# liamliaw/medical-image-segmentation-with-visual-prompts

Measured on AMD Instinct MI355X. Metric: 3D volumes/sec (96^3, bf16) training step, higher is better.
Workload: dtype bf16; 1 GPU; cfg1: swin_unetr downstream, 1-ch 96^3, batch 4/GPU, window (7, 7, 7), enc_prompt=False, dec_prompt=False, dropout 0.0, random-init weights; global_batch=4, parallelism=dp1, launch=eager (one C-ABI call per kernel)

## Files before the change

### medical-image-segmentation-with-visual-prompts_amd/csrc/swin_fwd.hip

```cpp
#include "swin_common.hpp"

template <int KS, bool CH12>
__global__ __launch_bounds__(256, 4) void k_swin_qkv_fwd(MivpSwinDesc d, const bf16_t* __restrict__ x,
                                                      const int* __restrict__ tok_src,
                                                      const float* __restrict__ ln_w, const float* __restrict__ ln_b,
                                                      const bf16_t* __restrict__ wqkv,
                                                      bf16_t* __restrict__ q, bf16_t* __restrict__ k,
                                                      bf16_t* __restrict__ v) {
    const int lane = threadIdx.x & 63, wave = __builtin_amdgcn_readfirstlane(threadIdx.x >> 6);
    const int r = lane & 15, g = lane >> 4;
    const int C = d.C, hd = C / d.heads;
    const long T = (long)d.B * d.P * d.Nqp;
    const long tile0 = ((long)blockIdx.x * 4 + wave) * 2;

    bf16x8 xb[2][KS];
    long bp[2];
    int slot[2];
    bool live[2];
#pragma unroll
    for (int u = 0; u < 2; ++u) {
        const long t = (tile0 + u) * 16 + r;
        live[u] = t < T;
        const unsigned tt = live[u] ? (unsigned)t : 0u;
        const unsigned bpu = tt / (unsigned)d.Nqp;
        bp[u] = bpu;
        slot[u] = (int)(tt - bpu * (unsigned)d.Nqp);
        const int pw = (int)(bpu % (unsigned)d.P);
        const long b = bpu / (unsigned)d.P;
        const int src = live[u] ? tok_src[pw * d.Nqp + slot[u]] : -2;
        float xs[KS][8];
        float sum = 0.f;
#pragma unroll
        for (int s = 0; s < KS; ++s) {
            const int c = 32 * s + 8 * g;
            if (src >= 0 && c < C) {
                bf16x8 raw = ld8(x + ((b * d.vol_in + src) * (long)C + c));
#pragma unroll
                for (int i = 0; i < 8; ++i) { xs[s][i] = (float)raw[i]; sum += xs[s][i]; }
            } else {
#pragma unroll
                for (int i = 0; i < 8; ++i) xs[s][i] = 0.f;
            }
        }
        const float mean = col_sum(sum) / (float)C;
        float var = 0.f;
#pragma unroll
        for (int s = 0; s < KS; ++s) {
            if (32 * s + 8 * g < C) {
#pragma unroll
                for (int i = 0; i < 8; ++i) { const float dv = xs[s][i] - mean; var += dv * dv; }
            }
        }
        const float rstd = rsqrtf(col_sum(var) / (float)C + d.ln_eps);
#pragma unroll
        for (int s = 0; s < KS; ++s) {
            const int c = 32 * s + 8 * g;
            bf16x8 y = zero8();
            if (src >= -1 && c < C) {
#pragma unroll
                for (int i = 0; i < 8; ++i) y[i] = (bf16_t)((xs[s][i] - mean) * rstd * ln_w[c + i] + ln_b[c + i]);
            }
            xb[u][s] = y;
        }
    }

    if constexpr (CH12) {
        const unsigned Nqp = (unsigned)d.Nqp;
        if (tile0 * 16 >= T) return;
        long chunk[2];
#pragma unroll
        for (int u = 0; u < 2; ++u) {
            const unsigned tt = (unsigned)((tile0 + u) * 16);
            const unsigned bpu = (unsigned)__builtin_amdgcn_readfirstlane((int)(tt / Nqp));
            chunk[u] = ((long)bpu * 4 * Nqp + (tt - bpu * Nqp)) * 12;
        }
        const int dl = lane < 48 ? lane : lane - 16, rq = dl / 3, gq = dl - 3 * rq;
        int src_addr[4];
        bool from_b[4];
#pragma unroll
        for (int h = 0; h < 4; ++h) {
            const int ch = 12 * h + 4 * gq;
            src_addr[h] = 4 * (rq + 16 * ((ch & 15) >> 2));
            from_b[h] = (ch >> 4) != ((12 * h) >> 4);
        }
#pragma unroll
        for (int sl = 0; sl < 3; ++sl) {
            const float sc = sl == 0 ? d.q_scale : (sl == 1 ? MIVP_LOG2E : 1.0f);
            u32x2 pk[3][2];
#pragma unroll
            for (int t = 0; t < 3; ++t) {
                f32x4 acc0 = fzero4(), acc1 = fzero4();
#pragma unroll
                for (int s = 0; s < KS; ++s) {
                    const char* fb = reinterpret_cast<const char*>(wqkv) + (size_t)(((3 * sl + t) * KS + s) * 1024);
                    const bf16x8 a = *reinterpret_cast<const bf16x8*>(fb + (unsigned)(16 * lane));
                    acc0 = mfma16(a, xb[0][s], acc0);
                    acc1 = mfma16(a, xb[1][s], acc1);
                }
                pk[t][0] = __builtin_bit_cast(u32x2, pack4(acc0 * sc));
                pk[t][1] = __builtin_bit_cast(u32x2, pack4(acc1 * sc));
            }
            bf16_t* base = sl == 0 ? q : (sl == 1 ? k : v);
#pragma unroll
            for (int h = 0; h < 4; ++h) {
                const int ta = (12 * h) >> 4, tb = (12 * h + 8) >> 4;
#pragma unroll
                for (int u = 0; u < 2; ++u) {
                    u32x2 piece;
                    piece[0] = (unsigned)__builtin_amdgcn_ds_bpermute(src_addr[h], (int)pk[ta][u][0]);
                    piece[1] = (unsigned)__builtin_amdgcn_ds_bpermute(src_addr[h], (int)pk[ta][u][1]);
                    if (tb != ta) {
                        const unsigned b0 = (unsigned)__builtin_amdgcn_ds_bpermute(src_addr[h], (int)pk[tb][u][0]);
                        const unsigned b1 = (unsigned)__builtin_amdgcn_ds_bpermute(src_addr[h], (int)pk[tb][u][1]);
                        piece[0] = from_b[h] ? b0 : piece[0];
                        piece[1] = from_b[h] ? b1 : piece[1];
                    }
                    char* cb = reinterpret_cast<char*>(base + (chunk[u] + (long)h * Nqp * 12));
                    *reinterpret_cast<u32x2*>(cb + (unsigned)(8 * dl)) = piece;
                }
            }
        }
        return;
    }
    const int n_out = 3 * C;
    const int n_tiles = (n_out + 15) / 16;
    const int per_split = (n_tiles + gridDim.y - 1) / gridDim.y;
    const int nt_begin = blockIdx.y * per_split;
    const int nt_end = nt_begin + per_split < n_tiles ? nt_begin + per_split : n_tiles;
    constexpr bool LDSW = KS >= 3;
    constexpr int PCS = (64 * KS + 255) / 256;
    __shared__ __attribute__((aligned(16))) char wsm[LDSW ? 2 * KS * 1024 : 16];
    using WR = OperandRows<32>;
    bf16x8 wreg[PCS];
    auto slab_fetch = [&](int nt) {
#pragma unroll
        for (int u = 0; u < PCS; ++u) {
            wreg[u] = ld8(wqkv + (long)nt * KS * 512 + 8 * min((int)threadIdx.x + 256 * u, 64 * KS - 1));
        }
    };
    auto slab_store = [&](int buf) {
#pragma unroll
        for (int u = 0; u < PCS; ++u) {
            *reinterpret_cast<bf16x8*>(wsm + buf * KS * 1024 + 16 * min((int)threadIdx.x + 256 * u, 64 * KS - 1)) = wreg[u];
        }
    };
    if (LDSW && nt_begin < nt_end) { slab_fetch(nt_begin); slab_store(0); __syncthreads(); }
    int o_sel = (16 * nt_begin + 4 * g) / C;
    int o_head = ((16 * nt_begin + 4 * g) - o_sel * C) / hd;
    int o_j0 = (16 * nt_begin + 4 * g) - o_sel * C - o_head * hd;
    for (int nt = nt_begin; nt < nt_end; ++nt) {
        f32x4 acc0 = fzero4(), acc1 = fzero4();
        const int nrow = 16 * nt + r;
        if (LDSW) {
            const int cur = (nt - nt_begin) & 1;
            if (nt + 1 < nt_end) slab_fetch(nt + 1);
            const char* slab = wsm + cur * KS * 1024;
#pragma unroll
            for (int s = 0; s < KS; ++s) {
                const bf16x8 a = *reinterpret_cast<const bf16x8*>(slab + s * 1024 + 16 * lane);
                acc0 = mfma16(a, xb[0][s], acc0);
                acc1 = mfma16(a, xb[1][s], acc1);
            }
            if (nt + 1 < nt_end) slab_store(cur ^ 1);
            __syncthreads();
        } else {
#pragma unroll
            for (int s = 0; s < KS; ++s) {
                const bf16x8 a = wfrag(wqkv, KS, nt, s, lane);
                acc0 = mfma16(a, xb[0][s], acc0);
                acc1 = mfma16(a, xb[1][s], acc1);
            }
        }
        const int n0 = 16 * nt + 4 * g;
        if (n0 < n_out) {
            while (o_j0 >= hd) { o_j0 -= hd; ++o_head; }
            while (o_head >= d.heads) { o_head -= d.heads; ++o_sel; }
            const int sel = o_sel, head = o_head, j0 = o_j0;
            o_j0 += 16;
            bf16_t* base = sel == 0 ? q : (sel == 1 ? k : v);
            const float sc = sel == 0 ? d.q_scale : (sel == 1 ? MIVP_LOG2E : 1.0f);
            if (live[0]) st4(base + ((bp[0] * d.heads + head) * d.Nqp + slot[0]) * (long)hd + j0, pack4(acc0 * sc));
            if (live[1]) st4(base + ((bp[1] * d.heads + head) * d.Nqp + slot[1]) * (long)hd + j0, pack4(acc1 * sc));
        }
    }
}

__global__ __launch_bounds__(256) void k_prompt_kv_fwd(MivpSwinDesc d, const float* __restrict__ prompt,
                                                       const float* __restrict__ ln_w, const float* __restrict__ ln_b,
                                                       const bf16_t* __restrict__ wqkv, bf16_t* __restrict__ kp,
                                                       bf16_t* __restrict__ vp, float* __restrict__ yln) {
    extern __shared__ __attribute__((aligned(16))) char smem[];
    float* y = reinterpret_cast<float*>(smem);
    float* red = y + d.C;
    const int t = blockIdx.x, C = d.C, hd = C / d.heads;
    const int tid = threadIdx.x;
    if (t >= d.Np) {
        for (int n = tid; n < 2 * C; n += 256) {
            const int sel = n / C, cc = n - sel * C, head = cc / hd, j = cc - head * hd;
            (sel == 0 ? kp : vp)[((long)head * d.Npp + t) * hd + j] = (bf16_t)0.0f;
        }
        return;
    }
    float part = 0.f;
    for (int c = tid; c < C; c += 256) part += prompt[(long)t * C + c];
    for (int o = 32; o > 0; o >>= 1) part += __shfl_xor(part, o);
    if ((tid & 63) == 0) red[tid >> 6] = part;
    __syncthreads();
    const float mean = (red[0] + red[1] + red[2] + red[3]) / (float)C;
    __syncthreads();
    part = 0.f;
    for (int c = tid; c < C; c += 256) { const float dv = prompt[(long)t * C + c] - mean; part += dv * dv; }
    for (int o = 32; o > 0; o >>= 1) part += __shfl_xor(part, o);
    if ((tid & 63) == 0) red[4 + (tid >> 6)] = part;
    __syncthreads();
    const float rstd = rsqrtf((red[4] + red[5] + red[6] + red[7]) / (float)C + d.ln_eps);
    for (int c = tid; c < C; c += 256) {
        const float yy = (prompt[(long)t * C + c] - mean) * rstd * ln_w[c] + ln_b[c];
        if (yln) yln[(long)t * C + c] = yy;
        y[c] = (float)(bf16_t)yy;
    }
    __syncthreads();
    for (int n = tid; n < 2 * C; n += 256) {
        const int sel = n / C, cc = n - sel * C;
        const bf16_t* wrow = wqkv + (long)((sel + 1) * C + cc) * C;
        float acc = 0.f;
        for (int c = 0; c < C; ++c) acc += y[c] * (float)wrow[c];
        const int head = cc / hd, j = cc - head * hd;
        (sel == 0 ? kp : vp)[((long)head * d.Npp + t) * hd + j] = (bf16_t)(sel == 0 ? acc * MIVP_LOG2E : acc);
    }
}

struct PromptKvJob {
    MivpSwinDesc d;
    const float* prompt; const float* ln_w; const float* ln_b; const bf16_t* wqkv; const float* ts;
    bf16_t* kp; bf16_t* vp; bf16_t* ka;
};
struct PromptKvJobs { PromptKvJob job[16]; };
__global__ __launch_bounds__(256) void k_prompt_kv_fwd_multi(PromptKvJobs jobs) {
    const PromptKvJob& jb = jobs.job[blockIdx.y];
    const MivpSwinDesc& d = jb.d;
    const int t = blockIdx.x;
    if (t >= d.Npp) return;
    extern __shared__ __attribute__((aligned(16))) char smem[];
    float* y = reinterpret_cast<float*>(smem);
    float* red = y + d.C;
    const int C = d.C, hd = C / d.heads;
    const int tid = threadIdx.x;
    const float* __restrict__ prompt = jb.prompt;
    if (t >= d.Np) {
        for (int n = tid; n < 2 * C; n += 256) {
            const int sel = n / C, cc = n - sel * C, head = cc / hd, j = cc - head * hd;
            (sel == 0 ? jb.kp : jb.vp)[((long)head * d.Npp + t) * hd + j] = (bf16_t)0.0f;
        }
        return;
    }
    for (int n = tid; n < d.heads * d.win[0]; n += 256) {
        const int head = n / d.win[0], a = n - head * d.win[0];
        jb.ka[((long)head * d.Nkp + d.Nqp + t) * d.augp + a] = (bf16_t)(jb.ts[(long)head * d.Np + t] * MIVP_LOG2E);
    }
    float part = 0.f;
    for (int c = tid; c < C; c += 256) part += prompt[(long)t * C + c];
    for (int o = 32; o > 0; o >>= 1) part += __shfl_xor(part, o);
    if ((tid & 63) == 0) red[tid >> 6] = part;
    __syncthreads();
    const float mean = (red[0] + red[1] + red[2] + red[3]) / (float)C;
    __syncthreads();
    part = 0.f;
    for (int c = tid; c < C; c += 256) { const float dv = prompt[(long)t * C + c] - mean; part += dv * dv; }
    for (int o = 32; o > 0; o >>= 1) part += __shfl_xor(part, o);
    if ((tid & 63) == 0) red[4 + (tid >> 6)] = part;
    __syncthreads();
    const float rstd = rsqrtf((red[4] + red[5] + red[6] + red[7]) / (float)C + d.ln_eps);
    for (int c = tid; c < C; c += 256)
        y[c] = (float)(bf16_t)((prompt[(long)t * C + c] - mean) * rstd * jb.ln_w[c] + jb.ln_b[c]);
    __syncthreads();
    for (int n = tid; n < 2 * C; n += 256) {
        const int sel = n / C, cc = n - sel * C;
        const bf16_t* wrow = jb.wqkv + (long)((sel + 1) * C + cc) * C;
        float acc = 0.f;
        for (int c = 0; c < C; ++c) acc += y[c] * (float)wrow[c];
        const int head = cc / hd, j = cc - head * hd;
        (sel == 0 ? jb.kp : jb.vp)[((long)head * d.Npp + t) * hd + j] = (bf16_t)(sel == 0 ? acc * MIVP_LOG2E : acc);
    }
}

__global__ __launch_bounds__(256) void k_relbias_aug(MivpSwinDesc d, const float* __restrict__ t_h,
                                                     const float* __restrict__ t_w, const float* __restrict__ t_d,
                                                     const float* __restrict__ ts, bf16_t* __restrict__ qa,
                                                     bf16_t* __restrict__ ka) {
    const int head = blockIdx.x;
    const int w0 = d.win[0], w1 = d.win[1], w2 = d.win[2];
    const int A = d.augp;
    const int chunk = blockIdx.y, nchunk = gridDim.y;
    if (head == d.heads) {
        for (int e = chunk * 256 + threadIdx.x; e < d.Nqp * A; e += nchunk * 256) {
            const int n = e / A, a = e - n * A;
            float val = 0.f;
            if (n < d.Nq) {
                const int i2 = n % w2, i1 = (n / w2) % w1, i0 = n / (w2 * w1);
                if (a < w0) val = (a == i0) ? 1.f : 0.f;
                else if (a < w0 + w1) val = (a - w0 == i1) ? 1.f : 0.f;
                else if (a < w0 + w1 + w2 - 1) val = (a - w0 - w1 == i2) ? 1.f : 0.f;
            }
            qa[e] = (bf16_t)val;
        }
        return;
    }
    const float* th = t_h + (long)head * (2 * w0 - 1);
    const float* tw = t_w + (long)head * (2 * w1 - 1);
    const float* td = t_d + (long)head * (2 * w2 - 1);
    for (int e = chunk * 256 + threadIdx.x; e < d.Nkp * A; e += nchunk * 256) {
        const int m = e / A, a = e - m * A;
        float val = 0.f;
        if (m < d.Nq) {
            const int k2 = m % w2, k1 = (m / w2) % w1, k0 = m / (w2 * w1);
            const float fold = td[k2 - (w2 - 1) + w2 - 1];
            if (a < w0) val = th[k0 - a + w0 - 1] + fold;
            else if (a < w0 + w1) val = tw[k1 - (a - w0) + w1 - 1];
            else if (a < w0 + w1 + w2 - 1) val = td[k2 - (a - w0 - w1) + w2 - 1] - fold;
        } else if (m >= d.Nqp && m < d.Nqp + d.Np) {
            if (a < w0) val = ts[(long)head * d.Np + (m - d.Nqp)];
        } else {
            if (a < w0) val = MIVP_PAD_KEY_BIAS;
        }
        ka[((long)head * d.Nkp + m) * A + a] = (bf16_t)(val * MIVP_LOG2E);
    }
}

__device__ __attribute__((aligned(16))) unsigned int g_attn_consts[4] = {0u, 0x00003F80u, 0u, 0u};

template <int DKS, bool DROP, bool MASKED>
constexpr int attn_fwd_occupancy() {
    if (DKS != 1) return 2;
    if (DROP) return 6;
    return MASKED ? 6 : 8;
}
template <int DKS, int DVT, int NW, int QT, bool DROP, bool ONES, bool MASKED, bool ZREF = false, bool BITS = false>
__global__ __launch_bounds__(64 * NW, (attn_fwd_occupancy<DKS, DROP, MASKED>())) void k_win_attn_fwd(MivpSwinDesc d, const bf16_t* __restrict__ q,
                                                         const bf16_t* __restrict__ k, const bf16_t* __restrict__ v,
                                                         const bf16_t* __restrict__ kp, const bf16_t* __restrict__ vp,
                                                         const bf16_t* __restrict__ qa, const bf16_t* __restrict__ ka,
                                                         const int* __restrict__ tok_rid, bf16_t* __restrict__ o,
                                                         float* __restrict__ lse, int xcd_remap,
                                                         const unsigned long long* __restrict__ mbits,
                                                         const unsigned char* __restrict__ cutw) {
    const uint32_t attn_key = drop_seed(d.attn_seed, d.seed_epoch), proj_key = drop_seed(d.proj_seed, d.seed_epoch);
    (void)attn_key; (void)proj_key;
    static_assert(!BITS || MASKED, "mask words belong to the masked kernels");
    extern __shared__ __attribute__((aligned(16))) char smem[];
    constexpr int DK = 32 * DKS;
    using KR = OperandRows<DK>;
    constexpr int KROW = KR::ROW;
    const int Nkp = d.Nkp, Nqp = d.Nqp;
    constexpr bool DMA = DKS == 1;
    static_assert(!DMA || DVT == 1, "the DMA-staged images are laid out for one k-step / one value tile");
    const int VROW = DMA ? 32 : (Nkp + 8) * 2;
    char* Kimg = smem;
    char* Vt = Kimg + (size_t)Nkp * KROW;
    uint8_t* ridk = reinterpret_cast<uint8_t*>(Vt + (DMA ? (size_t)Nkp * 32 : (size_t)(16 * DVT) * VROW));

    const int tid = threadIdx.x, lane = tid & 63;
    const int wave = __builtin_amdgcn_readfirstlane(tid >> 6);
    const int r = lane & 15, g = lane >> 4;
    const int C = d.C, heads = d.heads, hd = C / heads;
    long bph = blockIdx.x;
    if (xcd_remap) bph = (long)(blockIdx.x & 7) * (gridDim.x >> 3) + (blockIdx.x >> 3);
    const int head = (int)(bph % heads);
    const long bp = bph / heads;
    const int pw = (int)(bp % d.P);
    const int A = d.augp;
    const int hd4 = hd / 4, dk4 = DK / 4, a4 = A / 4;

    const bf16_t* kb = k + bph * (long)Nqp * hd;
    const bf16_t* vb = v + bph * (long)Nqp * hd;
    const bf16_t* kpb = d.Np > 0 ? kp + (long)head * d.Npp * hd : kb;
    const bf16_t* vpb = d.Np > 0 ? vp + (long)head * d.Npp * hd : vb;
    const bf16_t* kab = ka + (long)head * Nkp * A;
    const int n_prompt_rows = d.Np > 0 ? d.Npp : 0;
    if constexpr (DMA) {
        const char* zsrc = reinterpret_cast<const char*>(g_attn_consts);
        const int hd2 = hd >> 1, a2 = A >> 1;
        {
            const int sl = lane & 15, rowin = lane >> 4;
            const int ld = 4 * ((sl >> 2) ^ ((0 - wave) & 3)) + (sl & 3);
            const int kind = ld < hd2 ? 0 : (ld < hd2 + a2 ? 1 : 2);
            const int row0 = 4 * wave + rowin;
            const long stride = kind == 0 ? 64L * hd : (kind == 1 ? 64L * A : 0L);
            const char* src = kind == 0 ? reinterpret_cast<const char*>(kb) + ((long)row0 * hd + 2 * ld) * 2
                            : kind == 1 ? reinterpret_cast<const char*>(kab) + ((long)row0 * A + 2 * (ld - hd2)) * 2 : zsrc;
            int gi = wave;
            for (; gi < Nqp / 4; gi += NW) { glds4(src, Kimg + gi * 256); src += stride; }
            if (kind == 0) src = reinterpret_cast<const char*>(kpb) + ((long)(4 * gi + rowin - Nqp) * hd + 2 * ld) * 2;
            for (; gi < Nkp / 4; gi += NW) {
                const bool live = 4 * gi < Nqp + n_prompt_rows;
                glds4((kind == 0 && !live) ? zsrc : src, Kimg + gi * 256);
                src += stride;
            }
        }
        {
            const int sl = lane & 7, rowin = lane >> 3;
            const int row0 = 8 * wave + rowin;
            const bool fv = sl < hd2;
            const char* csrc = (ONES && sl == hd2) ? zsrc + 4 : zsrc;
            const long stride = fv ? 128L * hd : 0L;
            const char* src = fv ? reinterpret_cast<const char*>(vb) + ((long)row0 * hd + 2 * sl) * 2 : csrc;
            int gi = wave;
            for (; gi < Nqp / 8; gi += NW) { glds4(src, Vt + gi * 256); src += stride; }
            if (fv) src = reinterpret_cast<const char*>(vpb) + ((long)(8 * gi + rowin - Nqp) * hd + 2 * sl) * 2;
            for (; gi < Nkp / 8; gi += NW) {
                const bool live = 8 * gi < Nqp + n_prompt_rows;
                glds4((fv && !live) ? zsrc : src, Vt + gi * 256);
                src += stride;
            }
        }
    } else {
    {
        constexpr int RPP = 64 * NW / dk4;
        const int c4 = tid % dk4, row0 = tid / dk4;
        const bool from_k = c4 < hd4, from_a = !from_k && c4 < hd4 + a4;
        const bf16_t* src = from_k ? kb : kab;
        const uint32_t stride = from_k ? hd : A, coff = from_k ? 4 * c4 : 4 * (c4 - hd4);
        const int rows_main = from_k ? Nqp : (from_a ? Nkp : 0);
        for (int rowb = row0; rowb < Nkp; rowb += 4 * RPP) {
            bf16x4 vals[4];
#pragma unroll
            for (int i = 0; i < 4; ++i) {
// ... 232 lines not shown
                first = false;
            }
            bf16x8 vfr[DVT];
            if constexpr (DMA) {
                const char* vblk = Vt + (32 * u + 4 * g + (r >> 2)) * 32 + 8 * (r & 3);
                vfr[0] = cat44(tr_read(vblk), tr_read(vblk + 512));
            } else {
#pragma unroll
                for (int dd = 0; dd < DVT; ++dd) {
                    const char* vrow = Vt + (size_t)(16 * dd + r) * VROW;
                    vfr[dd] = cat44(*reinterpret_cast<const bf16x4*>(vrow + (32 * u + 4 * g) * 2),
                                    *reinterpret_cast<const bf16x4*>(vrow + (32 * u + 16 + 4 * g) * 2));
                }
            }
#pragma unroll
            for (int a = 0; a < QT; ++a) {
                float psum = 0.f;
#pragma unroll
                for (int hh = 0; hh < 2; ++hh)
#pragma unroll
                    for (int j = 0; j < 4; ++j) { const float pe = __builtin_amdgcn_exp2f(sv[a][hh][j]); sv[a][hh][j] = pe; if (!ONES) psum += pe; }
                if (!ONES) lsum[a] += psum;
                if (DROP) {
#pragma unroll
                    for (int hh = 0; hh < 2; ++hh) {
                        const int key0 = 16 * (2 * u + hh) + 4 * g;
                        const uint32_t pi = attn_pair(drow[a], key0);
                        const uint32_t h0 = drop_hash(pi, attn_key), h1 = drop_hash(pi + 1, attn_key);
                        sv[a][hh][0] = drop_keep(h0, 0, d.attn_drop_thr) ? sv[a][hh][0] : 0.f;
                        sv[a][hh][1] = drop_keep(h0, 1, d.attn_drop_thr) ? sv[a][hh][1] : 0.f;
                        sv[a][hh][2] = drop_keep(h1, 0, d.attn_drop_thr) ? sv[a][hh][2] : 0.f;
                        sv[a][hh][3] = drop_keep(h1, 1, d.attn_drop_thr) ? sv[a][hh][3] : 0.f;
                    }
                }
                bf16x8 pb;
                if (DROP) {
                    typedef float f32x2_t __attribute__((ext_vector_type(2)));
                    typedef __bf16 bf16x2_t __attribute__((ext_vector_type(2)));
                    u32x4 pk;
#pragma unroll
                    for (int hh = 0; hh < 2; ++hh)
#pragma unroll
                        for (int e = 0; e < 2; ++e) {
                            const f32x2_t two = {sv[a][hh][2 * e], sv[a][hh][2 * e + 1]};
                            pk[2 * hh + e] = __builtin_bit_cast(unsigned, __builtin_convertvector(two, bf16x2_t));
                        }
                    pb = __builtin_bit_cast(bf16x8, pk);
                } else {
                    pb = cat44(pack4(sv[a][0]), pack4(sv[a][1]));
                }
#pragma unroll
                for (int dd = 0; dd < DVT; ++dd) oacc[a][dd] = mfma16(vfr[dd], pb, oacc[a][dd]);
            }
        };
        const int nfull = nt_full / 2;
        auto walk = [&](auto mask_c, auto opt_c) {
            using first_opt = std::integral_constant<bool, ZREF && decltype(opt_c)::value>;
            if (nfull > 0) step(0, std::false_type{}, mask_c, first_opt{});
            else step(0, std::true_type{}, mask_c, first_opt{});
            int u = 1;
            if (decltype(opt_c)::value && !decltype(mask_c)::value) {
                for (; u + 1 < nfull; u += 2) { step(u, std::false_type{}, mask_c, opt_c); step(u + 1, std::false_type{}, mask_c, opt_c); }
            }
            for (; u < nfull; ++u) step(u, std::false_type{}, mask_c, opt_c);
            for (u = nfull > 1 ? nfull : 1; u < npairs; ++u) step(u, std::true_type{}, mask_c, opt_c);
        };
        auto row_sum_of = [&](int a) -> float {
            float ls = lsum[a];
            if (ONES) {
                const int dd1 = hd >> 4, e1 = hd & 3, g1 = (hd & 15) >> 2;
                float pick = 0.f;
#pragma unroll
                for (int dd = 0; dd < DVT; ++dd)
#pragma unroll
                    for (int e = 0; e < 4; ++e) pick = (dd == dd1 && e == e1) ? oacc[a][dd][e] : pick;
                ls = __shfl(pick, r + 16 * g1);
            } else {
                ls = col_sum(ls);
            }
            return ls;
        };
        if (MASKED && cut) walk(std::true_type{}, std::true_type{});
        else walk(std::false_type{}, std::true_type{});
        float ls_of[QT];
        {
            bool bad = false;
#pragma unroll
            for (int a = 0; a < QT; ++a) {
                ls_of[a] = row_sum_of(a);
                bad = bad || !(ls_of[a] < 1.2676506e30f) || (ZREF && !(ls_of[a] > 7.8886091e-31f));
            }
            if (__any(bad)) {
                reset();
                if (MASKED && cut) walk(std::true_type{}, std::false_type{});
                else walk(std::false_type{}, std::false_type{});
#pragma unroll
                for (int a = 0; a < QT; ++a) ls_of[a] = row_sum_of(a);
            }
        }
#pragma unroll
        for (int a = 0; a < QT; ++a) {
            if (a > 0 && qt0 + a >= nqt) continue;
            const float ls = ls_of[a];
            const float inv = (DROP ? d.attn_drop_scale : 1.0f) * __builtin_amdgcn_rcpf(ls);
#pragma unroll
            for (int dd = 0; dd < DVT; ++dd) {
                const int j0 = 16 * dd + 4 * g;
                if (j0 < hd) st4(ob + ((uint32_t)qrow[a] * C + j0), pack4(oacc[a][dd] * inv));
            }
            if (!ZREF && lse && g == 0) lse[bph * Nqp + qrow[a]] = (mrun[a] + __builtin_amdgcn_logf(ls)) * MIVP_LN2;
        }
    }
}

template <int CT>
__global__ __launch_bounds__(256, CT >= 12 ? 2 : (CT >= 6 ? 4 : 5)) void k_swin_proj_mlp_fwd(MivpSwinDesc d, const bf16_t* __restrict__ o,
                                                           const bf16_t* __restrict__ x,
                                                           const int* __restrict__ tok_src, const int* __restrict__ tok_dst,
                                                           const bf16_t* __restrict__ wproj, const float* __restrict__ bproj,
                                                           const float* __restrict__ ln_w, const float* __restrict__ ln_b,
                                                           const bf16_t* __restrict__ wmlp, const float* __restrict__ bmlp,
                                                           bf16_t* __restrict__ t1_out, bf16_t* __restrict__ y) {
    const uint32_t attn_key = drop_seed(d.attn_seed, d.seed_epoch), proj_key = drop_seed(d.proj_seed, d.seed_epoch);
    (void)attn_key; (void)proj_key;
    constexpr int KS = (CT + 1) / 2;
    constexpr bool LDSW = CT >= 6;
    constexpr int PCS = (64 * KS + 255) / 256;
    __shared__ __attribute__((aligned(16))) char wsm[LDSW ? 2 * KS * 1024 : 16];
    using WR = OperandRows<32>;
    const int lane = threadIdx.x & 63, wave = __builtin_amdgcn_readfirstlane(threadIdx.x >> 6);
    const int r = lane & 15, g = lane >> 4;
    const int C = d.C;
    const long T = (long)d.B * d.P * d.Nqp;
    const long t = ((long)blockIdx.x * 4 + wave) * 16 + r;
    const bool live = t < T;
    const unsigned tt = live ? (unsigned)t : 0u;
    const unsigned bpu = tt / (unsigned)d.Nqp;
    const long bp = bpu;
    const int slot = (int)(tt - bpu * (unsigned)d.Nqp);
    const int pw = (int)(bpu % (unsigned)d.P);
    const long b = bpu / (unsigned)d.P;
    const int src = sel(live, tok_src[pw * d.Nqp + slot], -2);
    const int dst = sel(live, tok_dst[pw * d.Nqp + slot], -1);
    bf16x8 wreg[PCS];
    auto slab_fetch = [&](const bf16_t* __restrict__ w, int nt) {
#pragma unroll
        for (int u = 0; u < PCS; ++u) {
            wreg[u] = ld8(w + (long)nt * KS * 512 + 8 * min((int)threadIdx.x + 256 * u, 64 * KS - 1));
        }
    };
    auto slab_store = [&](int buf) {
#pragma unroll
        for (int u = 0; u < PCS; ++u) {
            *reinterpret_cast<bf16x8*>(wsm + buf * KS * 1024 + 16 * min((int)threadIdx.x + 256 * u, 64 * KS - 1)) = wreg[u];
        }
    };

    bf16x8 ob[KS];
#pragma unroll
    for (int s = 0; s < KS; ++s) {
        const int c = 32 * s + 8 * g;
        ob[s] = keep_if(ld8(o + (tt * (long)C + min(c, C - 8))), live && c < C);
    }
    bf16x4 xraw[CT];
    const long xrow = (b * d.vol_in + max(src, 0)) * (long)C;
#pragma unroll
    for (int nt = 0; nt < CT; ++nt) xraw[nt] = ld4(x + xrow + min(16 * nt + 4 * g, C - 4));
    f32x4 t1[CT];
    float sum = 0.f;
    if (LDSW) { slab_fetch(wproj, 0); slab_store(0); __syncthreads(); }
#pragma unroll
    for (int nt = 0; nt < CT; ++nt) {
        f32x4 acc = fzero4();
        const int nrow = 16 * nt + r;
        if (LDSW) {
            if (nt + 1 < CT) slab_fetch(wproj, nt + 1);
            const char* slab = wsm + (nt & 1) * KS * 1024;
#pragma unroll
            for (int s = 0; s < KS; ++s)
                acc = mfma16(*reinterpret_cast<const bf16x8*>(slab + s * 1024 + 16 * lane), ob[s], acc);
            if (nt + 1 < CT) slab_store((nt + 1) & 1);
            __syncthreads();
        } else {
#pragma unroll
            for (int s = 0; s < KS; ++s) {
                acc = mfma16(wfrag(wproj, KS, nt, s, lane), ob[s], acc);
            }
        }
        const int n0 = 16 * nt + 4 * g;
        const f32x4 bp4 = *reinterpret_cast<const f32x4*>(bproj + min(n0, C - 4));
        if (n0 < C) {
            f32x4 sc;
            { const bf16x4 xv = keep_if(xraw[nt], src >= 0); for (int j = 0; j < 4; ++j) sc[j] = (float)xv[j]; }
            f32x4 keep = {1.f, 1.f, 1.f, 1.f};
            if (d.proj_drop_thr) {
                const uint32_t pi = (uint32_t)((tt * C + n0) >> 1);
                const uint32_t h0 = drop_hash(pi, proj_key), h1 = drop_hash(pi + 1, proj_key);
                keep[0] = drop_keep(h0, 0, d.proj_drop_thr) ? d.proj_drop_scale : 0.f;
                keep[1] = drop_keep(h0, 1, d.proj_drop_thr) ? d.proj_drop_scale : 0.f;
                keep[2] = drop_keep(h1, 0, d.proj_drop_thr) ? d.proj_drop_scale : 0.f;
                keep[3] = drop_keep(h1, 1, d.proj_drop_thr) ? d.proj_drop_scale : 0.f;
            }
#pragma unroll
            for (int j = 0; j < 4; ++j) {
                const float val = (float)(bf16_t)((acc[j] + bp4[j]) * keep[j] + sc[j]);
                acc[j] = val;
                sum += val;
            }
            if (t1_out && live) st4(t1_out + (tt * (long)C + n0), pack4(acc));
        } else {
            acc = fzero4();
        }
        t1[nt] = acc;
    }
    const float mean = col_sum(sum) / (float)C;
    float var = 0.f;
#pragma unroll
    for (int nt = 0; nt < CT; ++nt) {
        if (16 * nt + 4 * g < C) {
#pragma unroll
            for (int j = 0; j < 4; ++j) { const float dv = t1[nt][j] - mean; var += dv * dv; }
        }
    }
    const float rstd = rsqrtf(col_sum(var) / (float)C + d.ln_eps);
    bf16x4 y2[2 * KS];
#pragma unroll
    for (int nt = 0; nt < 2 * KS; ++nt) {
        bf16x4 yy = zero4();
        if (nt < CT) {
            const int n0 = 16 * nt + 4 * g;
            const f32x4 w4 = *reinterpret_cast<const f32x4*>(ln_w + min(n0, C - 4));
            const f32x4 b4 = *reinterpret_cast<const f32x4*>(ln_b + min(n0, C - 4));
#pragma unroll
            for (int j = 0; j < 4; ++j) yy[j] = (bf16_t)((t1[nt][j] - mean) * rstd * w4[j] + b4[j]);
            yy = keep_if(yy, n0 < C);
        }
        y2[nt] = yy;
    }
    if (LDSW) { slab_fetch(wmlp, 0); slab_store(0); __syncthreads(); }
#pragma unroll
    for (int mt = 0; mt < CT; ++mt) {
        f32x4 acc = fzero4();
        const int nrow = 16 * mt + r;
        if (LDSW) {
            if (mt + 1 < CT) slab_fetch(wmlp, mt + 1);
            const char* slab = wsm + (mt & 1) * KS * 1024;
#pragma unroll
            for (int s = 0; s < KS; ++s) {
                acc = mfma16(*reinterpret_cast<const bf16x8*>(slab + s * 1024 + 16 * lane), cat44(y2[2 * s], y2[2 * s + 1]), acc);
            }
            if (mt + 1 < CT) slab_store((mt + 1) & 1);
            __syncthreads();
        } else {
#pragma unroll
            for (int s = 0; s < KS; ++s) {
                acc = mfma16(wfrag(wmlp, KS, mt, s, lane), cat44(y2[2 * s], y2[2 * s + 1]), acc);
            }
        }
        const int n0 = 16 * mt + 4 * g;
        const f32x4 bm4 = *reinterpret_cast<const f32x4*>(bmlp + min(n0, C - 4));
        if (n0 < C && dst >= 0) {
#pragma unroll
            for (int j = 0; j < 4; ++j) acc[j] += t1[mt][j] + bm4[j];
            st4(y + ((b * d.vol_out + dst) * (long)C + n0), pack4(acc));
        }
    }
}

static int swin_common_checks(const MivpSwinDesc* d) {
    MIVP_REQUIRE(d != nullptr);
    MIVP_REQUIRE(d->B > 0 && d->C > 0 && d->heads > 0 && d->P > 0);
    MIVP_REQUIRE(d->C % 8 == 0 && d->C % d->heads == 0 && (d->C / d->heads) % 4 == 0);
    MIVP_REQUIRE(d->Nqp % 16 == 0 && d->Nqp >= d->Nq && d->Nqp - d->Nq < 16);
    MIVP_REQUIRE((long)d->B * d->P * d->Nqp < (1L << 31));
    MIVP_REQUIRE(d->Npp % 16 == 0 && d->Npp >= d->Np);
    MIVP_REQUIRE(d->Nkp % 32 == 0 && d->Nkp >= d->Nqp + d->Npp);
    MIVP_REQUIRE(d->augp % 4 == 0 && d->augp >= d->aug);
    MIVP_REQUIRE(d->aug == d->win[0] + d->win[1] + d->win[2] - 1);
    MIVP_REQUIRE(d->Nq == d->win[0] * d->win[1] * d->win[2]);
    return MIVP_OK;
}

extern "C" int mivp_swin_qkv_fwd(const MivpSwinDesc* d, const void* x, const int32_t* tok_src, const float* ln_w,
                                 const float* ln_b, const void* wqkv, void* q, void* k, void* v,
                                 mivp_stream_t stream) {
    int rc = swin_common_checks(d);
    if (rc) return rc;
    MIVP_REQUIRE(x && tok_src && ln_w && ln_b && wqkv && q && k && v);
    if (mivp_tok_wide_supported(d)) return mivp_tok_wide_qkv_fwd(d, x, tok_src, ln_w, ln_b, wqkv, q, k, v, (hipStream_t)stream);
    const long T = (long)d->B * d->P * d->Nqp;
    const unsigned gx = (unsigned)((T + 127) / 128);
    const int KS = (d->C + 31) / 32;
    const int n_tiles = (3 * d->C + 15) / 16;
    int nsplit = (int)((4096 + 4L * gx - 1) / (4L * gx));
    if (nsplit > n_tiles / 3) nsplit = n_tiles / 3;
    if (nsplit < 1) nsplit = 1;
    const dim3 grid(gx, (unsigned)nsplit);
    hipStream_t st = (hipStream_t)stream;
    const bool ch12 = d->C == 48 && d->heads == 4 && nsplit == 1 && d->Nqp % 32 == 0;
    auto launch = [&](auto kern) {
        hipLaunchKernelGGL(kern, grid, dim3(256), 0, st, *d, (const bf16_t*)x, tok_src, ln_w, ln_b, (const bf16_t*)wqkv,
                           (bf16_t*)q, (bf16_t*)k, (bf16_t*)v);
    };
    if (ch12) launch(k_swin_qkv_fwd<2, true>);
    else if (!for_tile_count<1, 2, 3, 4, 6>(KS, [&](auto ks) { launch(k_swin_qkv_fwd<decltype(ks)::value, false>); })) {
        mivp_set_error("swin_qkv_fwd: C/32 not in {1,2,3,4,6}");
        return MIVP_EUNSUPPORTED;
    }
    return mivp_check_launch("swin_qkv_fwd");
}

extern "C" int mivp_prompt_kv_fwd(const MivpSwinDesc* d, const float* prompt, const float* ln_w, const float* ln_b,
                                  const void* wqkv, void* kp, void* vp, float* yln, mivp_stream_t stream) {
    int rc = swin_common_checks(d);
    if (rc) return rc;
    MIVP_REQUIRE(d->Np > 0 && prompt && ln_w && ln_b && wqkv && kp && vp);
    hipLaunchKernelGGL(k_prompt_kv_fwd, dim3(d->Npp), dim3(256), (d->C + 8) * sizeof(float), (hipStream_t)stream, *d,
                       prompt, ln_w, ln_b, (const bf16_t*)wqkv, (bf16_t*)kp, (bf16_t*)vp, yln);
    return mivp_check_launch("prompt_kv_fwd");
}

extern "C" int mivp_prompt_kv_fwd_multi(int32_t n, const MivpSwinDesc* d, const float* const* prompt, const float* const* ln_w,
                                        const float* const* ln_b, const void* const* wqkv, const float* const* ts,
                                        void* const* kp, void* const* vp, void* const* ka, mivp_stream_t stream) {
    MIVP_REQUIRE(n > 0 && n <= 16 && d && prompt && ln_w && ln_b && wqkv && ts && kp && vp && ka);
    PromptKvJobs jobs;
    int rows = 0;
    size_t lds = 0;
    for (int i = 0; i < n; ++i) {
        int rc = swin_common_checks(&d[i]);
        if (rc) return rc;
        MIVP_REQUIRE(d[i].Np > 0 && prompt[i] && ln_w[i] && ln_b[i] && wqkv[i] && ts[i] && kp[i] && vp[i] && ka[i]);
        jobs.job[i] = PromptKvJob{d[i], prompt[i], ln_w[i], ln_b[i], (const bf16_t*)wqkv[i], ts[i], (bf16_t*)kp[i], (bf16_t*)vp[i],
                                  (bf16_t*)ka[i]};
        rows = d[i].Npp > rows ? d[i].Npp : rows;
        const size_t need = (d[i].C + 8) * sizeof(float);
        lds = need > lds ? need : lds;
    }
    hipLaunchKernelGGL(k_prompt_kv_fwd_multi, dim3(rows, n), dim3(256), lds, (hipStream_t)stream, jobs);
    return mivp_check_launch("prompt_kv_fwd_multi");
}

extern "C" int mivp_relbias_aug(const MivpSwinDesc* d, const float* t_h, const float* t_w, const float* t_d,
                                const float* ts, void* qa, void* ka, mivp_stream_t stream) {
    int rc = swin_common_checks(d);
    if (rc) return rc;
    MIVP_REQUIRE(t_h && t_w && t_d && qa && ka);
    MIVP_REQUIRE(d->Np == 0 || ts != nullptr);
    hipLaunchKernelGGL(k_relbias_aug, dim3(d->heads + 1, 8), dim3(256), 0, (hipStream_t)stream, *d, t_h, t_w, t_d, ts,
                       (bf16_t*)qa, (bf16_t*)ka);
    return mivp_check_launch("relbias_aug");
}

template <int DKS, int DVT, int NW, int QT, bool BITS>
static int launch_attn_fwd_cfg(const MivpSwinDesc* d, const void* q, const void* k, const void* v, const void* kp,
                               const void* vp, const void* qa, const void* ka, const int32_t* tok_rid, void* o, float* lse,
                               const unsigned long long* mask_words, const unsigned char* cut_flags, hipStream_t st) {
    const size_t krow = OperandRows<32 * DKS>::ROW, vrow = (d->Nkp + 8) * 2;
    constexpr bool DMA = DKS == 1;
    const size_t lds = (size_t)d->Nkp * krow + (DMA ? (size_t)d->Nkp * 32 : (size_t)16 * DVT * vrow) + (size_t)d->Nkp;
    if (lds > 160 * 1024) { mivp_set_error("win_attn_fwd: LDS image exceeds 160 KiB"); return MIVP_EUNSUPPORTED; }
    const bool ones = !d->attn_drop_thr && (d->C / d->heads) < 16 * DVT;
    const bool msk = d->has_mask != 0;
    const bool zref = lse == nullptr && !d->attn_drop_thr;
    auto kern = d->attn_drop_thr
        ? (msk ? k_win_attn_fwd<DKS, DVT, NW, QT, true, false, true, false, BITS> : k_win_attn_fwd<DKS, DVT, NW, QT, true, false, false, false, false>)
        : ones ? (zref ? (msk ? k_win_attn_fwd<DKS, DVT, NW, QT, false, true, true, true, BITS> : k_win_attn_fwd<DKS, DVT, NW, QT, false, true, false, true, false>)
                       : (msk ? k_win_attn_fwd<DKS, DVT, NW, QT, false, true, true, false, BITS> : k_win_attn_fwd<DKS, DVT, NW, QT, false, true, false, false, false>))
               : (zref ? (msk ? k_win_attn_fwd<DKS, DVT, NW, QT, false, false, true, true, BITS> : k_win_attn_fwd<DKS, DVT, NW, QT, false, false, false, true, false>)
                       : (msk ? k_win_attn_fwd<DKS, DVT, NW, QT, false, false, true, false, BITS> : k_win_attn_fwd<DKS, DVT, NW, QT, false, false, false, false, false>));
    if (lds > 64 * 1024) {
        hipError_t e = hipFuncSetAttribute(reinterpret_cast<const void*>(kern), hipFuncAttributeMaxDynamicSharedMemorySize, (int)lds);
        if (e != hipSuccess) { mivp_set_error(hipGetErrorString(e)); return MIVP_ELAUNCH; }
    }
    const unsigned grid = (unsigned)((long)d->B * d->P * d->heads);
    const int xcd_remap = (grid % 8 == 0 && grid >= 64) ? 1 : 0;
    hipLaunchKernelGGL(kern, dim3(grid), dim3(64 * NW), lds, st, *d, (const bf16_t*)q, (const bf16_t*)k, (const bf16_t*)v,
                       (const bf16_t*)kp, (const bf16_t*)vp, (const bf16_t*)qa, (const bf16_t*)ka, tok_rid, (bf16_t*)o, lse, xcd_remap,
                       mask_words, cut_flags);
    return mivp_check_launch("win_attn_fwd");
}

template <int DKS, int DVT>
static int launch_attn_fwd(const MivpSwinDesc* d, const void* q, const void* k, const void* v, const void* kp,
                           const void* vp, const void* qa, const void* ka, const int32_t* tok_rid, void* o, float* lse,
                           const unsigned long long* mw, const unsigned char* cf, hipStream_t st) {
    const bool bits = d->has_mask && mw != nullptr && cf != nullptr;
    if (bits) return launch_attn_fwd_cfg<DKS, DVT, 8, 1, true>(d, q, k, v, kp, vp, qa, ka, tok_rid, o, lse, mw, cf, st);
    return launch_attn_fwd_cfg<DKS, DVT, 8, 1, false>(d, q, k, v, kp, vp, qa, ka, tok_rid, o, lse, mw, cf, st);
}

int mivp_attn_tile_config(const MivpSwinDesc* d, int* dks, int* nt) {
    const int hd = d->C / d->heads;
    const int dk = hd + d->augp;
    int ks = (dk + 31) / 32;
    const int vt = (hd + 15) / 16;
    if (vt > ks) ks = vt;
    *dks = ks;
    *nt = d->Nkp / 16;
    if (ks > 3) return MIVP_EUNSUPPORTED;
    return MIVP_OK;
}

extern "C" int mivp_win_attn_fwd(const MivpSwinDesc* d, const void* q, const void* k, const void* v, const void* kp,
                                 const void* vp, const void* qa, const void* ka, const int32_t* tok_rid, void* o,
                                 float* lse, const uint64_t* mask_words, const uint8_t* cut_flags, mivp_stream_t stream) {
    int rc = swin_common_checks(d);
    if (rc) return rc;
    MIVP_REQUIRE(q && k && v && qa && ka && o);
    MIVP_REQUIRE(d->Np == 0 || (kp && vp));
    MIVP_REQUIRE(!d->has_mask || tok_rid);
    int dks, nt;
    if (mivp_attn_tile_config(d, &dks, &nt)) { mivp_set_error("win_attn_fwd: head_dim / key count outside the instantiated set"); return MIVP_EUNSUPPORTED; }
    hipStream_t st = (hipStream_t)stream;
    const unsigned long long* mw = reinterpret_cast<const unsigned long long*>(mask_words);
    if (dks == 1) return launch_attn_fwd<1, 1>(d, q, k, v, kp, vp, qa, ka, tok_rid, o, lse, mw, cut_flags, st);
    if (dks == 2) return launch_attn_fwd<2, 2>(d, q, k, v, kp, vp, qa, ka, tok_rid, o, lse, mw, cut_flags, st);
    return launch_attn_fwd<3, 3>(d, q, k, v, kp, vp, qa, ka, tok_rid, o, lse, mw, cut_flags, st);
}

extern "C" int mivp_swin_proj_mlp_fwd(const MivpSwinDesc* d, const void* o, const void* x, const int32_t* tok_src,
                                      const int32_t* tok_dst, const void* wproj, const float* bproj, const float* ln_w,
                                      const float* ln_b, const void* wmlp, const float* bmlp, void* t1, void* y,
                                      mivp_stream_t stream) {
    int rc = swin_common_checks(d);
    if (rc) return rc;
    MIVP_REQUIRE(o && x && tok_src && tok_dst && wproj && bproj && ln_w && ln_b && wmlp && bmlp && y);
    const long T = (long)d->B * d->P * d->Nqp;
    const unsigned grid = (unsigned)((T + 63) / 64);
    const int CT = (d->C + 15) / 16;
    hipStream_t st = (hipStream_t)stream;
    if (mivp_tok_rows_supported(d))
        return mivp_tok_wide_proj_mlp_fwd(d, o, x, tok_src, tok_dst, wproj, bproj, ln_w, ln_b,
                                          (const bf16_t*)wmlp + mivp_tok_natural_offset(d->C), bmlp, t1, y, st);
    const bool known = for_tok16_ct(CT, [&](auto ct) {
        hipLaunchKernelGGL((k_swin_proj_mlp_fwd<decltype(ct)::value>), dim3(grid), dim3(256), 0, st, *d, (const bf16_t*)o,
                           (const bf16_t*)x, tok_src, tok_dst, (const bf16_t*)wproj, bproj, ln_w, ln_b, (const bf16_t*)wmlp, bmlp,
                           (bf16_t*)t1, (bf16_t*)y);
    });
    if (!known) { mivp_set_error("swin_proj_mlp_fwd: C/16 not in {1,2,3,4,6,8,12}"); return MIVP_EUNSUPPORTED; }
    return mivp_check_launch("swin_proj_mlp_fwd");
}
```

Before: 1685 volumes/s.

## Process two tile pairs per wave in C=48 QKV forward with hoisted weights

The C=48, 4-head QKV projection path now has each wave handle two pairs of 16-token tiles instead of one. Weights for each of q/k/v are loaded once into registers and reused across both pairs. All token gathers are issued up front, before the LayerNorm and MFMA work, to increase memory-level parallelism. The grid shrinks accordingly, at the cost of more register pressure and fewer waves, which can hurt occupancy or tail balance.

```diff
diff --git a/medical-image-segmentation-with-visual-prompts_amd/csrc/swin_fwd.hip b/medical-image-segmentation-with-visual-prompts_amd/csrc/swin_fwd.hip
--- a/medical-image-segmentation-with-visual-prompts_amd/csrc/swin_fwd.hip
+++ b/medical-image-segmentation-with-visual-prompts_amd/csrc/swin_fwd.hip
@@ -1,4 +1,167 @@
 #include "swin_common.hpp"
+
+constexpr int QKV_C48_PAIRS = 2;
+
+struct C48Tile { int src; long xrow, chunk; };
+MIVP_DEV C48Tile c48_tile(const MivpSwinDesc& d, const int* __restrict__ tok_src, long tile, int r) {
+    const unsigned Nqp = (unsigned)d.Nqp, tt = (unsigned)(tile * 16);
+    const unsigned bpu = (unsigned)__builtin_amdgcn_readfirstlane((int)(tt / Nqp));
+    const unsigned slot0 = tt - bpu * Nqp;
+    const unsigned b = (unsigned)__builtin_amdgcn_readfirstlane((int)(bpu / (unsigned)d.P));
+    const unsigned pw = bpu - b * (unsigned)d.P;
+    C48Tile t;
+    t.src = tok_src[pw * Nqp + slot0 + (unsigned)r];
+    t.xrow = (long)b * d.vol_in;
+    t.chunk = ((long)bpu * 4 * Nqp + slot0) * 12;
+    return t;
+}
+
+MIVP_DEV void c48_gather(const bf16_t* __restrict__ x, const C48Tile& t, int g, bf16x8 (&raw)[2]) {
+    const long row = (t.xrow + max(t.src, 0)) * 48L;
+    raw[0] = ld8(x + (row + 8 * g));
+    raw[1] = ld8(x + (row + min(32 + 8 * g, 40)));
+}
+
+MIVP_DEV void c48_ln(const MivpSwinDesc& d, const bf16x8 (&raw)[2], int src, int g, const float* __restrict__ ln_w,
+                     const float* __restrict__ ln_b, bf16x8 (&xb)[2]) {
+    const int C = d.C;
+    float xs[2][8];
+    float sum = 0.f;
+#pragma unroll
+    for (int s = 0; s < 2; ++s) {
+        const bool ok = src >= 0 && 32 * s + 8 * g < C;
+#pragma unroll
+        for (int i = 0; i < 8; ++i) { xs[s][i] = sel(ok, (float)raw[s][i], 0.f); sum += xs[s][i]; }
+    }
+    const float mean = col_sum(sum) / (float)C;
+    float var = 0.f;
+#pragma unroll
+    for (int s = 0; s < 2; ++s) {
+        const bool in = 32 * s + 8 * g < C;
+#pragma unroll
+        for (int i = 0; i < 8; ++i) {
+#pragma clang fp contract(off)
+            const float dv = xs[s][i] - mean;
+            const float sq = dv * dv;
+            var = sel(in, var + sq, var);
+        }
+    }
+    const float rstd = rsqrtf(col_sum(var) / (float)C + d.ln_eps);
+#pragma unroll
+    for (int s = 0; s < 2; ++s) {
+        const int c = min(32 * s + 8 * g, 40);
+        const bool ok = src >= -1 && 32 * s + 8 * g < C;
+        bf16x8 y;
+#pragma unroll
+        for (int i = 0; i < 8; ++i) y[i] = (bf16_t)__builtin_fmaf((xs[s][i] - mean) * rstd, ln_w[c + i], ln_b[c + i]);
+        xb[s] = keep_if(y, ok);
+    }
+}
+
+struct C48Route { int dl, src_addr[4]; bool from_b[4]; };
+MIVP_DEV C48Route c48_route(int lane) {
+    C48Route rt;
+    rt.dl = lane < 48 ? lane : lane - 16;
+    const int rq = rt.dl / 3, gq = rt.dl - 3 * rq;
+#pragma unroll
+    for (int h = 0; h < 4; ++h) {
+        const int ch = 12 * h + 4 * gq;
+        rt.src_addr[h] = 4 * (rq + 16 * ((ch & 15) >> 2));
+        rt.from_b[h] = (ch >> 4) != ((12 * h) >> 4);
+    }
+    return rt;
+}
+
+MIVP_DEV void c48_wthird(const bf16_t* __restrict__ wqkv, int sl, int lane, bf16x8 (&w)[3][2]) {
+#pragma unroll
+    for (int t = 0; t < 3; ++t) {
+#pragma unroll
+        for (int s = 0; s < 2; ++s) {
+            const char* fb = reinterpret_cast<const char*>(wqkv) + (size_t)(((3 * sl + t) * 2 + s) * 1024);
+            w[t][s] = *reinterpret_cast<const bf16x8*>(fb + (unsigned)(16 * lane));
+        }
+    }
+}
+
+MIVP_DEV void c48_third(const MivpSwinDesc& d, const bf16x8 (&w)[3][2], const bf16x8 (&xb)[2][2], float sc, bf16_t* base,
+                        const long (&chunk)[2], const C48Route& rt) {
+    const unsigned Nqp = (unsigned)d.Nqp;
+    u32x2 pk[3][2];
+#pragma unroll
+    for (int t = 0; t < 3; ++t) {
+        f32x4 acc0 = fzero4(), acc1 = fzero4();
+#pragma unroll
+        for (int s = 0; s < 2; ++s) {
+            acc0 = mfma16(w[t][s], xb[0][s], acc0);
+            acc1 = mfma16(w[t][s], xb[1][s], acc1);
+        }
+        pk[t][0] = __builtin_bit_cast(u32x2, pack4(acc0 * sc));
+        pk[t][1] = __builtin_bit_cast(u32x2, pack4(acc1 * sc));
+    }
+#pragma unroll
+    for (int h = 0; h < 4; ++h) {
+        const int ta = (12 * h) >> 4, tb = (12 * h + 8) >> 4;
+#pragma unroll
+        for (int u = 0; u < 2; ++u) {
+            u32x2 piece;
+            piece[0] = (unsigned)__builtin_amdgcn_ds_bpermute(rt.src_addr[h], (int)pk[ta][u][0]);
+            piece[1] = (unsigned)__builtin_amdgcn_ds_bpermute(rt.src_addr[h], (int)pk[ta][u][1]);
+            if (tb != ta) {
+                const unsigned b0 = (unsigned)__builtin_amdgcn_ds_bpermute(rt.src_addr[h], (int)pk[tb][u][0]);
+                const unsigned b1 = (unsigned)__builtin_amdgcn_ds_bpermute(rt.src_addr[h], (int)pk[tb][u][1]);
+                piece[0] = rt.from_b[h] ? b0 : piece[0];
+                piece[1] = rt.from_b[h] ? b1 : piece[1];
+            }
+            char* cb = reinterpret_cast<char*>(base + (chunk[u] + (long)h * Nqp * 12));
+            *reinterpret_cast<u32x2*>(cb + (unsigned)(8 * rt.dl)) = piece;
+        }
+    }
+}
+
+template <int R>
+MIVP_DEV void qkv_c48_tiles(const MivpSwinDesc& d, const bf16_t* __restrict__ x, const int* __restrict__ tok_src,
+                            const float* __restrict__ ln_w, const float* __restrict__ ln_b, const bf16_t* __restrict__ wqkv,
+                            bf16_t* __restrict__ q, bf16_t* __restrict__ k, bf16_t* __restrict__ v) {
+    const int lane = threadIdx.x & 63, wave = __builtin_amdgcn_readfirstlane(threadIdx.x >> 6);
+    const int r = lane & 15, g = lane >> 4;
+    const long pairs = ((long)d.B * d.P * d.Nqp) >> 5;
+    const long pair0 = ((long)blockIdx.x * 4 + wave) * R;
+    if (pair0 >= pairs) return;
+    const int n = (int)min((long)R, pairs - pair0);
+    C48Tile tl[R][2];
+#pragma unroll
+    for (int j = 0; j < R; ++j) {
+#pragma unroll
+        for (int u = 0; u < 2; ++u) tl[j][u] = c48_tile(d, tok_src, (pair0 + min(j, n - 1)) * 2 + u, r);
+    }
+    bf16x8 raw[R][2][2];
+#pragma unroll
+    for (int j = 0; j < R; ++j) {
+#pragma unroll
+        for (int u = 0; u < 2; ++u) c48_gather(x, tl[j][u], g, raw[j][u]);
+    }
+    bf16x8 xb[R][2][2];
+#pragma unroll
+    for (int j = 0; j < R; ++j) {
+#pragma unroll
+        for (int u = 0; u < 2; ++u) c48_ln(d, raw[j][u], tl[j][u].src, g, ln_w, ln_b, xb[j][u]);
+    }
+    const C48Route rt = c48_route(lane);
+#pragma unroll
+    for (int sl = 0; sl < 3; ++sl) {
+        bf16x8 w[3][2];
+        c48_wthird(wqkv, sl, lane, w);
+        const float sc = sl == 0 ? d.q_scale : (sl == 1 ? MIVP_LOG2E : 1.0f);
+        bf16_t* base = sl == 0 ? q : (sl == 1 ? k : v);
+#pragma unroll
+        for (int j = 0; j < R; ++j) {
+            if (j < n) {
+                const long chunk[2] = {tl[j][0].chunk, tl[j][1].chunk};
+                c48_third(d, w, xb[j], sc, base, chunk, rt);
+            }
+        }
+    }
+}
 
 template <int KS, bool CH12>
 __global__ __launch_bounds__(256, 4) void k_swin_qkv_fwd(MivpSwinDesc d, const bf16_t* __restrict__ x,
@@ -7,6 +170,10 @@
                                                       const bf16_t* __restrict__ wqkv,
                                                       bf16_t* __restrict__ q, bf16_t* __restrict__ k,
                                                       bf16_t* __restrict__ v) {
+    if constexpr (CH12) {
+        qkv_c48_tiles<QKV_C48_PAIRS>(d, x, tok_src, ln_w, ln_b, wqkv, q, k, v);
+        return;
+    }
     const int lane = threadIdx.x & 63, wave = __builtin_amdgcn_readfirstlane(threadIdx.x >> 6);
     const int r = lane & 15, g = lane >> 4;
     const int C = d.C, hd = C / d.heads;
@@ -64,64 +231,6 @@
         }
     }
 
-    if constexpr (CH12) {
-        const unsigned Nqp = (unsigned)d.Nqp;
-        if (tile0 * 16 >= T) return;
-        long chunk[2];
-#pragma unroll
-        for (int u = 0; u < 2; ++u) {
-            const unsigned tt = (unsigned)((tile0 + u) * 16);
-            const unsigned bpu = (unsigned)__builtin_amdgcn_readfirstlane((int)(tt / Nqp));
-            chunk[u] = ((long)bpu * 4 * Nqp + (tt - bpu * Nqp)) * 12;
-        }
-        const int dl = lane < 48 ? lane : lane - 16, rq = dl / 3, gq = dl - 3 * rq;
-        int src_addr[4];
-        bool from_b[4];
-#pragma unroll
-        for (int h = 0; h < 4; ++h) {
-            const int ch = 12 * h + 4 * gq;
-            src_addr[h] = 4 * (rq + 16 * ((ch & 15) >> 2));
-            from_b[h] = (ch >> 4) != ((12 * h) >> 4);
-        }
-#pragma unroll
-        for (int sl = 0; sl < 3; ++sl) {
-            const float sc = sl == 0 ? d.q_scale : (sl == 1 ? MIVP_LOG2E : 1.0f);
-            u32x2 pk[3][2];
-#pragma unroll
-            for (int t = 0; t < 3; ++t) {
-                f32x4 acc0 = fzero4(), acc1 = fzero4();
-#pragma unroll
-                for (int s = 0; s < KS; ++s) {
-                    const char* fb = reinterpret_cast<const char*>(wqkv) + (size_t)(((3 * sl + t) * KS + s) * 1024);
-                    const bf16x8 a = *reinterpret_cast<const bf16x8*>(fb + (unsigned)(16 * lane));
-                    acc0 = mfma16(a, xb[0][s], acc0);
-                    acc1 = mfma16(a, xb[1][s], acc1);
-                }
-                pk[t][0] = __builtin_bit_cast(u32x2, pack4(acc0 * sc));
-                pk[t][1] = __builtin_bit_cast(u32x2, pack4(acc1 * sc));
-            }
-            bf16_t* base = sl == 0 ? q : (sl == 1 ? k : v);
-#pragma unroll
-            for (int h = 0; h < 4; ++h) {
-                const int ta = (12 * h) >> 4, tb = (12 * h + 8) >> 4;
-#pragma unroll
-                for (int u = 0; u < 2; ++u) {
-                    u32x2 piece;
-                    piece[0] = (unsigned)__builtin_amdgcn_ds_bpermute(src_addr[h], (int)pk[ta][u][0]);
-                    piece[1] = (unsigned)__builtin_amdgcn_ds_bpermute(src_addr[h], (int)pk[ta][u][1]);
-                    if (tb != ta) {
-                        const unsigned b0 = (unsigned)__builtin_amdgcn_ds_bpermute(src_addr[h], (int)pk[tb][u][0]);
-                        const unsigned b1 = (unsigned)__builtin_amdgcn_ds_bpermute(src_addr[h], (int)pk[tb][u][1]);
-                        piece[0] = from_b[h] ? b0 : piece[0];
-                        piece[1] = from_b[h] ? b1 : piece[1];
-                    }
-                    char* cb = reinterpret_cast<char*>(base + (chunk[u] + (long)h * Nqp * 12));
-                    *reinterpret_cast<u32x2*>(cb + (unsigned)(8 * dl)) = piece;
-                }
-            }
-        }
-        return;
-    }
     const int n_out = 3 * C;
     const int n_tiles = (n_out + 15) / 16;
     const int per_split = (n_tiles + gridDim.y - 1) / gridDim.y;
@@ -960,8 +1069,12 @@
         hipLaunchKernelGGL(kern, grid, dim3(256), 0, st, *d, (const bf16_t*)x, tok_src, ln_w, ln_b, (const bf16_t*)wqkv,
                            (bf16_t*)q, (bf16_t*)k, (bf16_t*)v);
     };
-    if (ch12) launch(k_swin_qkv_fwd<2, true>);
-    else if (!for_tile_count<1, 2, 3, 4, 6>(KS, [&](auto ks) { launch(k_swin_qkv_fwd<decltype(ks)::value, false>); })) {
+    if (ch12) {
+        const long pairs = T / 32;
+        const unsigned gp = (unsigned)((pairs + 4 * QKV_C48_PAIRS - 1) / (4 * QKV_C48_PAIRS));
+        hipLaunchKernelGGL((k_swin_qkv_fwd<2, true>), dim3(gp), dim3(256), 0, st, *d, (const bf16_t*)x, tok_src, ln_w, ln_b,
+                           (const bf16_t*)wqkv, (bf16_t*)q, (bf16_t*)k, (bf16_t*)v);
+    } else if (!for_tile_count<1, 2, 3, 4, 6>(KS, [&](auto ks) { launch(k_swin_qkv_fwd<decltype(ks)::value, false>); })) {
         mivp_set_error("swin_qkv_fwd: C/32 not in {1,2,3,4,6}");
         return MIVP_EUNSUPPORTED;
     }
```

Result: faster. 1714 volumes/s, median of 6 (+1.7%).
